# NVlabs/geomapnet

Hardware: AMD Instinct MI355X
Metric: images/sec MapNet ResNet-34 256x341 T=3 train step (higher is better)
Workload: dtype f16 (MFMA operands f16, f32 accumulate; forward conv operands as f16 pairs hi + lo, 3 MFMAs per product; backward 1 MFMA per product)

## Files before the change

### geomapnet_amd/_binding.py

```python
import ctypes as C
import os

_HERE = os.path.dirname(os.path.abspath(__file__))
LIB_PATH = os.path.join(_HERE, "libmapnet_hip.so")

c_void = C.c_void_p
c_f = C.c_float
c_i = C.c_int
c_i64 = C.c_int64


class Entry(C.Structure):
    _fields_ = [("name", C.c_char * 96), ("offset", c_i64), ("numel", c_i64), ("ndim", C.c_int32),
                ("shape", C.c_int32 * 4), ("is_buffer", C.c_int32), ("is_int64", C.c_int32), ("ohwi", C.c_int32),
                ("stage", C.c_int32)]


class Config(C.Structure):
    _fields_ = [("mode", C.c_int32), ("dtype", C.c_int32), ("windows", C.c_int32), ("T", C.c_int32), ("H", C.c_int32),
                ("W", C.c_int32), ("feat_dim", C.c_int32), ("filter_nans", C.c_int32), ("loss_scale", c_f),
                ("eps_mode", C.c_int32)]


class GatherGeom(C.Structure):
# ... 3 lines not shown

_PROTOS = {
    "mn_last_error": (C.c_char_p, []),
    "mn_backend": (C.c_char_p, []),
    "mn_model_entries": (c_i, [c_i]),
    "mn_model_entry": (c_i, [c_i, c_i, C.POINTER(Entry)]),
    "mn_model_param_floats": (c_i64, [c_i]),
    "mn_model_buffer_bytes": (c_i64, [c_i]),
    "mn_plan_bytes": (c_i64, [C.POINTER(Config)]),
    "mn_create": (c_void, [C.POINTER(Config), c_void, c_void, c_void, c_void, c_void]),
    "mn_destroy": (None, [c_void]),
    "mn_set_learn_flags": (c_i, [c_void, c_i, c_i]),
    "mn_set_loss_fn": (c_i, [c_void, c_i, c_f, c_i, c_f]),
    "mn_set_optim": (c_i, [c_void, c_f, c_f, c_f, c_f, c_f, c_f]),
    "mn_set_optim_method": (c_i, [c_void, c_i, c_i]),
    "mn_set_step_count": (c_i, [c_void, c_i64]),
    "mn_get_step_count": (c_i64, [c_void]),
    "mn_stuck_overflow_steps": (c_i64, [c_void]),
    "mn_set_loss_host": (c_i, [c_void, c_void]),
    "mn_wait_loss": (c_i, [c_void]),
    "mn_set_loss_scale": (c_i, [c_void, c_f, c_i]),
    "mn_get_loss_scale": (c_i, [c_void, C.POINTER(c_f), C.POINTER(c_i64)]),
    "mn_debug_tensor": (c_i, [c_void, C.c_char_p, C.POINTER(c_void), C.POINTER(c_i64), C.POINTER(C.c_int32)]),
    "mn_set_dropout": (c_i, [c_void, c_f, C.c_uint64]),
    "mn_set_dropout_calls": (c_i, [c_void, C.c_uint32]),
    "mn_set_input_u8": (c_i, [c_void, c_i, C.POINTER(c_f), C.POINTER(c_f)]),
    "mn_set_color_jitter": (c_i, [c_void, c_f, c_f, c_f, c_f, C.c_uint64]),
    "mn_set_color_jitter_calls": (c_i, [c_void, C.c_uint32]),
    "mn_input_resize_bytes": (c_i64, [C.POINTER(Config), c_i, c_i]),
    "mn_set_input_resize": (c_i, [c_void, c_i, c_i, c_void, c_i64]),
    "mn_forward": (c_i, [c_void, c_void, c_void, c_i, c_void]),
    "mn_input_grad": (c_i, [c_void, c_void, c_void, c_void, c_void, c_void, c_void]),
    "mn_loss": (c_i, [c_void, c_void, c_void, c_void, c_void]),
    "mn_train_step": (c_i, [c_void, c_void, c_void, c_void, c_void, c_void]),
    "mn_train_forward_loss": (c_i, [c_void, c_void, c_void, c_void, c_void, c_void]),
    "mn_train_backward_stage": (c_i, [c_void, c_i, c_void]),
    "mn_grad_bucket": (c_i, [c_void, c_i, C.POINTER(c_i64), C.POINTER(c_i64)]),
    "mn_optim_step": (c_i, [c_void, c_f, c_void]),
    "mn_grad_bucket_pack_bf16": (c_i, [c_void, c_i, c_void, c_void]),
    "mn_grad_bucket_unpack_bf16": (c_i, [c_void, c_i, c_void, c_void]),
    "mn_params_changed": (c_i, [c_void]),
    "mn_set_profiling": (c_i, [c_void, c_i]),
    "mn_last_kernel_ms": (c_i, [c_void, c_i, C.POINTER(c_f), C.POINTER(c_i)]),
    "mn_op_igemm": (c_i, [c_i, C.POINTER(GatherGeom), c_void, c_void, c_void, c_i, c_void, c_void, c_i, c_void, c_void,
                          c_f, c_void, c_void]),
    "mn_op_igemm_grid_m": (c_i, [c_i]),
    "mn_op_wgrad": (c_i, [c_i, C.POINTER(GatherGeom), c_void, c_i, c_void, c_void, c_i, c_void, c_f, c_i, c_void, c_void]),
    "mn_op_wgrad_ws_floats": (c_i64, []),
    "mn_op_wgrad_ws": (c_i, [c_i, C.POINTER(GatherGeom), c_void, c_i, c_void, c_void, c_i, c_f, c_void, c_i64, c_void, c_void]),
    "mn_op_conv_halo_pp": (c_i, [C.POINTER(GatherGeom), c_void, c_void, c_void, c_i, c_void, c_i, c_i, c_void, c_void, c_void, c_f,
                                 c_i, c_void]),
    "mn_op_conv_halo_pp_h2gates": (c_i, [C.POINTER(GatherGeom), c_void, c_void, c_void, c_i, c_void, c_i, c_i, c_void, c_void, c_void,
                                         c_f, c_i, c_void]),
    "mn_op_conv_halo_h2": (c_i, [C.POINTER(GatherGeom), c_void, c_void, c_void, c_i, c_void, c_i, c_void]),
    "mn_op_conv_dgrad": (c_i, [c_i, c_i, c_i, c_i, c_i, c_i, c_i, c_i, c_i, c_void, c_void, c_void, c_void, c_void, c_void, c_i,
                               c_void, c_void]),
    "mn_op_stem_conv": (c_i, [c_void, c_void, c_void, c_void, c_i, c_i, c_i, c_i, c_i, c_void]),
    "mn_op_stem_conv_x3": (c_i, [c_void, c_void, c_void, c_void, c_i, c_i, c_i, c_i, c_i, c_void]),
    "mn_op_dense": (c_i, [c_void, c_void, c_void, c_void, c_i, c_i, c_i, c_i, c_void]),
    "mn_op_dense_wgrad": (c_i, [c_void, c_void, c_void, c_void, c_i, c_i, c_i, c_f, c_void]),
    "mn_op_head_wgrad": (c_i, [c_void, c_void, c_void, c_void, c_void, c_void, c_i, c_i, c_f, c_i, c_void]),
    "mn_op_stem_bwd": (c_i, [c_void, c_void, c_void, c_void, c_void, c_void, c_void, c_void, c_void, c_i, c_void, c_void, c_void,
                             c_void, c_void, c_i, c_i, c_i, c_i, c_f, c_void]),
    "mn_op_stem_bwd_pregated": (c_i, [c_void, c_void, c_void, c_void, c_void, c_void, c_void, c_void, c_void, c_i, c_void, c_void,
                                      c_void, c_void, c_void, c_i, c_i, c_i, c_i, c_f, c_void]),
    "mn_op_oihw_to_ohwi": (c_i, [c_void, c_void, c_i, c_i, c_i, c_i, c_i, c_void]),
    "mn_op_criterion": (c_i, [c_i, c_i, c_i, c_void, c_void, c_void, c_void, c_void, c_void, c_void, c_f, c_void]),
    "mn_op_criterion_fn": (c_i, [c_i, c_i, c_i, c_void, c_void, c_void, c_void, c_void, c_void, c_void, c_f, c_i, c_f, c_i, c_f,
                                 c_void]),
    "mn_op_calc_vos": (c_i, [c_void, c_i, c_i, c_void, c_void, c_void, c_void]),
    "mn_pgo_optimize": (c_i, [c_void, c_void, c_void, c_void, c_i, c_i, c_i, C.c_double, C.c_double, C.c_double,
                              C.c_double, c_i, c_void]),
    "mn_op_adam": (c_i, [c_void, c_void, c_void, c_void, c_i64, c_i64, c_f, c_f, c_f, c_f, c_f, c_i64, c_f, c_f, c_void,
                         c_i, c_void]),
    "mn_op_optim": (c_i, [c_i, c_i, c_void, c_void, c_void, c_void, c_i64, c_i64, c_f, c_f, c_f, c_f, c_f, c_i64, c_f, c_f, c_void,
                          c_i, c_void]),
    "mn_op_bn_train_fwd": (c_i, [c_i, c_void, c_i64, c_i, c_void, c_void, c_void, c_void, c_void, c_void, c_void, c_i,
                                 c_void, c_f, c_f, c_void, c_void]),
    "mn_op_bn_bwd": (c_i, [c_i, c_void, c_void, c_void, c_i64, c_i, c_void, c_void, c_void, c_void, c_void, c_void, c_void,
                           c_void, c_f, c_void]),
    "mn_op_bn_train_fwd_h2": (c_i, [c_void, c_i64, c_i, c_void, c_void, c_void, c_void, c_void, c_void, c_void, c_i, c_void, c_void,
                                    c_f, c_f, c_void, c_void]),
    "mn_op_bn_bwd_rows": (c_i, [c_i, c_void, c_void, c_void, c_i64, c_i, c_void, c_void, c_void, c_void, c_void, c_void, c_void,
                                c_void, c_void, c_i, c_f, c_void]),
    "mn_op_bn_relu_maxpool_h2": (c_i, [c_void, c_void, c_void, c_void, c_void, c_i, c_i, c_i, c_i, c_void]),
    "mn_op_avgpool_fwd_h2": (c_i, [c_void, c_void, c_i, c_i, c_i, c_void]),
    "mn_op_avgpool_bwd": (c_i, [c_i, c_void, c_void, c_void, c_i, c_i, c_i, c_void]),
    "mn_op_widen_f16": (c_i, [c_void, c_void, c_i64, c_void]),
    "mn_op_maxpool_fwd": (c_i, [c_i, c_void, c_void, c_void, c_i, c_i, c_i, c_i, c_void]),
    "mn_op_maxpool_bwd": (c_i, [c_i, c_void, c_void, c_void, c_i, c_i, c_i, c_i, c_void]),
    "mn_op_occupy": (c_i, [c_i, c_i, c_f, c_void, c_void, c_i64, c_i, c_void]),
    "mn_op_color_jitter": (c_i, [c_void, c_void, c_void, c_void, c_i, c_i, c_i, C.POINTER(c_f), C.c_uint64, C.c_uint32,
                                 C.POINTER(c_f), C.POINTER(c_f), c_void]),
    "mn_op_resize_u8": (c_i, [c_void, c_void, c_void, c_i, c_i, c_i, c_i, c_i, c_void]),
    "mn_op_resize_work_bytes": (c_i64, [c_i, c_i, c_i, c_i]),
    "mn_op_resize_tile": (c_i, [c_i, c_i, c_i, c_i, C.POINTER(c_i), C.POINTER(c_i)]),
    "mn_op_stem_dgrad": (c_i, [c_i, c_void, c_void, c_void, c_i, c_i, c_i, c_f, c_void]),
    "mn_op_bn_eval_bwd": (c_i, [c_i, c_void, c_void, c_void, c_void, c_i64, c_i, c_void]),
    "mn_op_saliency": (c_i, [c_void, c_void, c_void, c_void, c_i, c_i, c_i, c_void]),
    "mn_op_saliency_work_floats": (c_i64, [c_i]),
}

SYMBOLS = tuple(_PROTOS)


class MapNetHipError(RuntimeError):
# ... 53 lines not shown
```

### geomapnet_amd/csrc/knobs.h

```cpp
#pragma once
#include <stdlib.h>

namespace mn {

constexpr int kKnobUnset = -0x7fffffff;

struct Knobs {
  bool deterministic = false;
  int fuse_stem = 1;
  bool wgrad_stream = true;
  bool early_fork = true;
  int wgrad_sched = kKnobUnset;
  int wgrad_early_stages = kKnobUnset;
  int wgrad_defer_stages = kKnobUnset;
  int wgrad_tail = 1;
  int scale_growth = 2000;

  int igemm_config = 0;
  int igemm_halo = 2;
  int halo384 = 1;
  int halo_a1 = 1;
  bool h2_halo256 = false;
  bool wgrad_fused = true;
  int stem_wgs = 0;
  int halo_pp_wgs = 256;
  int halo_h2_wgs = 256;

#ifdef MN_ABLATION_BUILD
  int ablate = 0;
  int wgf_ablate = 0;
  int halo_ablate = 0;
  int halo_pp_ablate = 0;
  int halo_h2_ablate = 0;
  int abl_skip_finalize = 0;
  bool abl_skip_wgf = false;
  bool wgf_skip_reduce = false;
#endif
};

namespace knob_env {
inline int integer(const char* name, int dflt) {
  const char* e = getenv(name);
  return e ? atoi(e) : dflt;
}
inline bool on_unless_0(const char* name) { return integer(name, 1) != 0; }
inline bool present(const char* name) { return getenv(name) != nullptr; }
}

inline Knobs& knobs_storage() {
  static Knobs k;
  return k;
}
inline const Knobs& knobs() { return knobs_storage(); }

inline void load_knobs() {
  using namespace knob_env;
  Knobs k;
  k.deterministic = integer("MN_DETERMINISTIC", 0) != 0;
  k.fuse_stem = integer("MN_FUSE_STEM", k.fuse_stem);
  k.wgrad_stream = on_unless_0("MN_WGRAD_STREAM");
  k.early_fork = on_unless_0("MN_EARLY_FORK");
  k.wgrad_sched = integer("MN_WGRAD_SCHED", kKnobUnset);
  k.wgrad_early_stages = integer("MN_WGRAD_EARLY_STAGES", kKnobUnset);
  k.wgrad_defer_stages = integer("MN_WGRAD_DEFER_STAGES", kKnobUnset);
  k.wgrad_tail = integer("MN_WGRAD_TAIL", k.wgrad_tail);
  k.scale_growth = integer("MN_SCALE_GROWTH", k.scale_growth);
  k.igemm_config = integer("MN_IGEMM_CONFIG", k.igemm_config);
  k.igemm_halo = integer("MN_IGEMM_HALO", k.igemm_halo);
  k.halo384 = integer("MN_HALO384", k.halo384);
  k.halo_a1 = integer("MN_HALO_A1", k.halo_a1);
  k.h2_halo256 = integer("MN_H2_HALO256", 0) != 0;
  k.wgrad_fused = on_unless_0("MN_WGRAD_FUSED");
  k.stem_wgs = integer("MN_STEM_WGS", k.stem_wgs);
  k.halo_pp_wgs = integer("MN_HALO_PP_WGS", k.halo_pp_wgs);
  k.halo_h2_wgs = integer("MN_HALO_H2_WGS", k.halo_h2_wgs);
#ifdef MN_ABLATION_BUILD
  k.ablate = integer("MN_ABLATE", 0);
  k.wgf_ablate = integer("MN_WGF_ABLATE", 0);
  k.halo_ablate = integer("MN_HALO_ABLATE", 0);
  k.halo_pp_ablate = integer("MN_HALO_PP_ABLATE", 0);
  k.halo_h2_ablate = integer("MN_HALO_H2_ABLATE", 0);
  k.abl_skip_finalize = integer("MN_ABL_SKIP_FINALIZE", 0);
  k.abl_skip_wgf = present("MN_ABL_SKIP_WGF");
  k.wgf_skip_reduce = present("MN_WGF_SKIP_REDUCE");
#endif
  knobs_storage() = k;
}

struct WgradSchedule {
  int sched, early_stages, defer_stages;
};
inline WgradSchedule resolve_wgrad_schedule(const Knobs& k, bool f16_family, bool per_stage) {
  WgradSchedule r;
  r.sched = k.wgrad_sched != kKnobUnset ? k.wgrad_sched : !k.early_fork ? 0 : f16_family ? 1 : 2;
  r.early_stages = k.wgrad_early_stages != kKnobUnset ? k.wgrad_early_stages : per_stage ? 13 : 15;
  r.defer_stages = k.wgrad_defer_stages != kKnobUnset ? k.wgrad_defer_stages : per_stage ? 2 : 0;
  return r;
}

}
```

### geomapnet_amd/csrc/net.hip

```cpp
#include "../../include/mapnet_hip.h"

#include <cmath>
#include <cstring>
#include <deque>
#include <memory>
#include <string>
#include <vector>

#include "common.h"
#include "criterion.h"
#include "elementwise.h"
#include "elementwise_h2.h"
#include "head.h"
#include "jitter.h"
#include "resize.h"
#include "knobs.h"
#include "dense.h"
#include "igemm.h"
#include "dgrad.h"
#include "halo_pp.h"
#include "input_grad.h"
#include "layout.h"
#include "optim.h"
#include "pool.h"
#include "stem.h"
#include "stem_bwd.h"
#include "util.h"
#include "wgrad.h"

using namespace mn;

static const Layout& layout_for(int feat_dim) {
  static thread_local std::unique_ptr<Layout> cache;
  if (!cache || cache->feat_dim != feat_dim) cache.reset(new Layout(feat_dim));
  return *cache;
}
extern "C" int mn_model_entries(int feat_dim) { return (int)layout_for(feat_dim).entries.size(); }
extern "C" int mn_model_entry(int feat_dim, int idx, mn_entry* out) {
  const Layout& L = layout_for(feat_dim);
  if (idx < 0 || idx >= (int)L.entries.size()) return fail("mn_model_entry: index out of range");
  *out = L.entries[idx];
  return 0;
}
extern "C" int64_t mn_model_param_floats(int feat_dim) { return layout_for(feat_dim).param_floats; }
extern "C" int64_t mn_model_buffer_bytes(int feat_dim) { return layout_for(feat_dim).buffer_bytes; }

namespace {

struct Bump {
  size_t cur = 0;
  size_t take(size_t bytes) {
    size_t o = cur;
    cur += (bytes + 255) & ~(size_t)255;
    return o;
  }
};

struct KernelTimer {
  bool enabled = false;
  struct Pair {
    hipEvent_t a, b;
    int cat;
  };
  std::deque<Pair> pool;
  size_t used = 0;
  float ms[4] = {0, 0, 0, 0};
  int launches[4] = {0, 0, 0, 0};
  Pair* begin(int cat, hipStream_t s) {
    if (!enabled) return nullptr;
    if (used == pool.size()) {
      Pair p;
      hipEventCreate(&p.a);
      hipEventCreate(&p.b);
// ... 554 lines not shown
  }
  void launch_repack(int first_block, int n_blocks, int n_jobs, hipStream_t s) {
    void (*kernel)(const RepackJob*, int, const float*, int) = repack_all_kernel<T>;
    if constexpr (DT == MN_F32) {
      if (md.wf == FMT_H2Q)
        kernel = repack_all_kernel<float, true, true, true>;
      else if (md.wf == FMT_H2 && md.wd == FMT_F16)
        kernel = repack_all_kernel<float, true, true>;
      else if (md.wf == FMT_H2)
        kernel = repack_all_kernel<float, true>;
    }
    hipLaunchKernelGGL(kernel, dim3(n_blocks), dim3(256), 0, s, (const RepackJob*)repack_jobs, n_jobs, (const float*)params,
                       first_block);
  }

  BnParams bn_params(const Unit& u) {
    BnParams p;
    p.gamma = params + u.bp.gamma;
    p.beta = params + u.bp.beta;
    p.running_mean = (float*)buffers + u.bp.rm;
    p.running_var = (float*)buffers + u.bp.rv;
    p.num_batches_tracked = (long long*)(buffers + u.bp.nbt);
    p.mean = u.mean;
    p.invstd = u.invstd;
    p.eps = 1e-5f;
    p.momentum = 0.1f;
    return p;
  }
  static Epilogue plain_epilogue(void* out, int ldc) {
    Epilogue ep;
    ep.out = out; ep.ldc = ldc; ep.stats = nullptr; ep.bias = nullptr; ep.relu = 0; ep.res = nullptr; ep.res_gate = nullptr;
    ep.alpha = 1.f;
    return ep;
  }
  static GatherGeom dense_geom(int M, int N, int K) {
    GatherGeom g;
    g.B = M; g.Hi = 1; g.Wi = 1; g.C = K; g.P = 1; g.Q = 1; g.R = 1; g.S = 1; g.mul_p = 1; g.mul_q = 1; g.rsign = 1;
    g.ssign = 1; g.off_h = 0; g.off_w = 0; g.div = 1; g.M = M; g.N = N; g.K = K;
    return g;
  }
  Epilogue stats_epilogue(Unit& u, int training) {
    Epilogue ep = plain_epilogue(u.y, u.cp.cout);
    if (training) {
      ep.stats_accum = u.accum_f;
      ep.stats_rows = u.rows_f;
    }
    return ep;
  }
  void conv_bn_stats(Unit& u, const T* x, int training, hipStream_t s) {
    const Epilogue ep = stats_epilogue(u, training);
    auto* tp = timer.begin(0, s);
    if (md.pairs())
      launch_igemm_h2(u.gf, (const half*)x, (const half*)u.wf, ep, s, (const half*)zero_page, md.act == FMT_H2Q);
    else if (halo_path(u.gf) && conv_halo_pp_applies(u.gf, ep))
      launch_conv_halo_pp(u.gf, (const half*)x, (const half*)u.wf, ep, s);
    else
      launch_igemm<T>(u.gf, x, u.wf, ep, s, (const T*)zero_page);
    timer.end(tp, s);
  }
  void stem_conv(int training, hipStream_t s) {
    double* const sums = training ? stem.accum_f : nullptr;
    auto* tp = timer.begin(0, s);
    if (DT == MN_F32 && md.mma_fwd == MMA_F16X3)
      launch_stem_conv_x3((const float*)xpad, (const float*)stem.wf, (float*)stem.y, sums, stem.rows_f, B, H, W, Wp, s);
    else if (DT == MN_F16)
      launch_stem_conv((const half*)xpad, (const half*)stem.wf, (half*)stem.y, sums, stem.rows_f, B, H, W, Wp, s);
    else
      launch_igemm<T>(stem.gf, xpad, stem.wf, stats_epilogue(stem, training), s, (const T*)zero_page);
    timer.end(tp, s);
  }
  bool halo_path(const GatherGeom& g) const { return md.act == FMT_F16 && conv_halo_applies(g); }
  void bn_finalize(Unit& u, hipStream_t s) {
#ifdef MN_ABLATION_BUILD
    const int skip_c = knobs().abl_skip_finalize;
    static long calls = 0;
    if (u.cp.cout <= skip_c && ++calls > 400) return;
#endif
    hipLaunchKernelGGL(bn_finalize_fwd_kernel, dim3(cdiv(u.cp.cout, kBnFinalizeChannels)), dim3(256), 0, s, (const double*)u.accum_f, (double)u.M,
                       bn_params(u), cur_training, u.coef_f, u.cp.cout, u.rows_f);
  }
  void bn_act(Unit& u, const T* res, int relu, T* out, hipStream_t s) {
    long np = u.M * u.cp.cout / VEC;
    bn_finalize(u, s);
    if (md.pairs()) {
      const long ni = u.M * u.cp.cout / 8;
      hipLaunchKernelGGL(bn_apply_h2_kernel, dim3(ew_grid(ni)), dim3(256), 0, s, (const float*)u.y, (const float*)u.coef_f,
                         (const half*)res, (half*)out, ni, u.cp.cout, relu, md.act == FMT_H2Q ? 1 : 0,
                         cur_training ? u.rec : (half*)nullptr, (const float*)u.mean, (const float*)u.invstd);
      return;
    }
    hipLaunchKernelGGL((bn_apply_kernel<T>), dim3(ew_grid(np)), dim3(256), 0, s, (const T*)u.y, (const float*)u.coef_f, res, out,
                       np, u.cp.cout, relu);
  }

  void launch_jitter_input(const unsigned char* images, half* x16, hipStream_t s) {
    launch_u8_jitter<T>(images, xpad, B, H, W, Hp, Wp, jitter_norm, x16, jitter_params(jit_range, jit_seed, jit_calls), jit_draws,
                        jit_partials, jit_mean, s);
    jit_calls += 1;
  }

  int forward(const void* images, float* poses_out, int training, hipStream_t s) override {
    return forward_impl(images, poses_out, training, false, s);
  }
  int forward_impl(const void* images, float* poses_out, int training, bool zero_grads, hipStream_t s) {
    if (jitter_on() && !input_u8)
      return fail("forward: ColorJitter (mn_set_color_jitter) needs uint8 input (mn_set_input_u8): fp32 frames arrive already "
                  "normalised, and ColorJitter must come before Normalize");
    if (resize_on && !input_u8)
// ... 109 lines not shown
    if (int e = forward_impl(images, poses_out, 1, true, s)) return e;
    cur_targets = targets;
    cur_loss = loss_out ? loss_out : loss_dev;
    return 0;
  }

  void bn_bwd(Unit& u, const T* g, hipStream_t s, bool self_gate = false) {
    float* const gamma = params + u.bp.gamma;
    const float* const sg_beta = self_gate ? params + u.bp.beta : nullptr;
    if (md.f16_bwd_on_pairs())
      launch_bn_bwd_rec((const half*)g, (const half*)u.rec, u.M, u.cp.cout, gamma, u.mean, u.invstd, grads + u.bp.gamma,
                        grads + u.bp.beta, (half*)u.gy, u.accum_b, u.coef_b, 1.f / cur_scale, s, self_gate, u.rows_b);
    else if (md.gy == FMT_H2)
      launch_bn_bwd_h2((const float*)g, (const float*)u.y, u.M, u.cp.cout, gamma, u.mean, u.invstd, grads + u.bp.gamma,
                       grads + u.bp.beta, (half*)u.gy, u.accum_b, u.coef_b, 1.f / cur_scale, s, sg_beta, u.rows_b);
    else
      launch_bn_bwd<T>(g, (const T*)nullptr, (const T*)u.y, u.M, u.cp.cout, gamma, u.mean, u.invstd, grads + u.bp.gamma,
                       grads + u.bp.beta, u.gy, u.accum_b, u.coef_b, 1.f / cur_scale, s, sg_beta, PoolGradSrc(), u.rows_b);
  }
  WgradArgs wgrad_args(Unit& u, const T* x) {
    WgradArgs a;
    a.g = u.gf; a.dY = u.gy; a.ldy = u.cp.cout; a.X = x; a.dW = grads + u.cp.w; a.ldw = u.ldw; a.colmap = u.colmap;
    a.g.mma = md.mma_bwd;
    a.alpha = 1.f / cur_scale; a.rows_per_split = 0;
    a.ws = wgf_ws; a.ws_floats = wgf_ws_floats;
    a.det = deterministic;
    return a;
  }
  static int wgrad_splits(const Unit& u) { return u.cp.cout >= 128 ? 512 : (u.M > 2000000 ? 2048 : 1024); }
  void conv_wgrad(Unit& u, const T* x, hipStream_t ws) {
    WgradArgs a = wgrad_args(u, x);
    auto* tp = timer.begin(1, ws);
    if (md.f16_bwd_on_pairs()) {
      a.g.mma = MMA_NATIVE;
      a.x_h2 = true;
      launch_wgrad<half>(a, wgrad_splits(u), ws, zero_page);
    } else if (md.gy == FMT_H2) {
      a.g.mma = MMA_H2;
      launch_wgrad<half>(a, wgrad_splits(u), ws, zero_page);
    } else {
      launch_wgrad<T>(a, wgrad_splits(u), ws, zero_page);
    }
    timer.end(tp, ws);
  }
  void conv_dgrad(Unit& u, T* gx, const T* res, hipStream_t s, const T* out_gate = nullptr) {
    Epilogue ep = plain_epilogue(gx, u.cp.cin);
    ep.res = res;
    ep.out_gate = out_gate;
    auto* tp = timer.begin(0, s);
    if (md.gy == FMT_H2) {
      launch_conv_dgrad<half>(u.dg, (const half*)u.gy, (const half*)u.wd, ep, s, (const half*)zero_page, parity_dgrad, true);
    } else if (md.gy == FMT_F16) {
      ep.gate_h2 = md.pairs();
      if (conv_halo_applies(u.dg.full) && conv_halo_pp_applies(u.dg.full, ep))
        launch_conv_halo_pp(u.dg.full, (const half*)u.gy, (const half*)u.wd, ep, s);
      else
        launch_conv_dgrad<half>(u.dg, (const half*)u.gy, (const half*)u.wd, ep, s, (const half*)zero_page, parity_dgrad);
    } else {
      launch_conv_dgrad<T>(u.dg, (const T*)u.gy, (const T*)u.wd, ep, s, (const T*)zero_page, parity_dgrad);
    }
    timer.end(tp, s);
  }
  void block_input_dgrad(Block& blk, const T* below, hipStream_t s) {
    if (blk.down) {
      conv_dgrad(blk.u1, blk.gx, nullptr, s, below);
      conv_dgrad(blk.ud, blk.gx, blk.gx, s, below);
    } else {
      conv_dgrad(blk.u1, blk.gx, blk.gout, s, below);
    }
  }
  void flush_wgrads(hipStream_t s) {
    if (pending_wgrads.empty()) return;
    hipStream_t ws = fork_wgrad(s);
    for (auto& p : pending_wgrads) conv_wgrad(*p.u, p.x, ws);
    pending_wgrads.clear();
  }
  void block_backward(Block& blk, hipStream_t s) {
    const T* bx = blk.x;
    const T* ba1 = blk.a1;
    const T* below = &blk == &blocks.front() ? (md.stem_bwd == STEM_TILES_ON_COPIES ? bx : nullptr) : bx;
    if (wgrad.sched == 2 || ((wgrad.defer_stages >> blk.stage) & 1)) {
      flush_wgrads(s);
      bn_bwd(blk.u2, blk.gout, s);
      conv_dgrad(blk.u2, blk.ga1, nullptr, s);
      pending_wgrads.push_back({&blk.u2, ba1});
      flush_wgrads(s);
      bn_bwd(blk.u1, blk.ga1, s, true);
      if (blk.down) bn_bwd(blk.ud, blk.gout, s);
      pending_wgrads.push_back({&blk.u1, bx});
      if (blk.down) pending_wgrads.push_back({&blk.ud, bx});
      block_input_dgrad(blk, below, s);
      return;
    }
    bn_bwd(blk.u2, blk.gout, s);
    const bool tail = blk.stage == 0 && !blk.down && (int)(&blk - &blocks[0]) < wgrad_tail;
    const bool early = wgrad.sched == 1 && !tail && ((wgrad.early_stages >> blk.stage) & 1);
    if (early) conv_wgrad(blk.u2, ba1, fork_wgrad(s));
    conv_dgrad(blk.u2, blk.ga1, nullptr, s);
    bn_bwd(blk.u1, blk.ga1, s, true);
    if (blk.down) bn_bwd(blk.ud, blk.gout, s);
    if (tail) {
      pending_wgrads.push_back({&blk.u2, ba1});
      pending_wgrads.push_back({&blk.u1, bx});
    } else {
      hipStream_t ws = fork_wgrad(s);
      if (!early) conv_wgrad(blk.u2, ba1, ws);
      conv_wgrad(blk.u1, bx, ws);
      if (blk.down) conv_wgrad(blk.ud, bx, ws);
// ... 584 lines not shown
```

### geomapnet_amd/csrc/ops.hip

```cpp
#include "../../include/mapnet_hip.h"

#include <string>

#include "common.h"
#include "criterion.h"
#include "elementwise.h"
#include "elementwise_h2.h"
#include "head.h"
#include "jitter.h"
#include "knobs.h"
#include "dense.h"
#include "igemm.h"
#include "dgrad.h"
#include "halo_pp.h"
#include "input_grad.h"
#include "optim.h"
#include "pgo.h"
#include "pool.h"
#include "rehearsal.h"
#include "resize.h"
#include "stem.h"
#include "stem_bwd.h"
#include "wgrad.h"
#include "util.h"

using namespace mn;

namespace mn {
thread_local std::string g_last_error;
}

extern "C" const char* mn_last_error(void) { return mn::g_last_error.c_str(); }

#ifndef MN_BACKEND_NAME
#define MN_BACKEND_NAME "hip"
#endif
extern "C" const char* mn_backend(void) { return MN_BACKEND_NAME; }

static void begin_op() {
  begin_call();
  load_knobs();
}

static GatherGeom to_geom(const mn_gather_geom* g) {
  GatherGeom r;
  r.B = g->B; r.Hi = g->Hi; r.Wi = g->Wi; r.C = g->C; r.P = g->P; r.Q = g->Q; r.R = g->R; r.S = g->S;
  r.mul_p = g->mul_p; r.mul_q = g->mul_q; r.rsign = g->rsign; r.ssign = g->ssign;
  r.off_h = g->off_h; r.off_w = g->off_w; r.div = g->div; r.M = g->M; r.N = g->N; r.K = g->K;
  return r;
}

static int check_geom(const GatherGeom& g, int dtype) {
  int vec = dtype == MN_F16 ? 8 : 4;
  if ((dtype == MN_DTYPE_F16X2 || dtype == MN_DTYPE_F16X2Q) && (g.C % 32 != 0 || g.N % 4 != 0))
    return fail("igemm: h2 operands need C % 32 == 0");
  if (g.C % vec != 0) return fail("igemm: C must be a multiple of the 16-byte piece");
  if (g.K != g.R * g.S * g.C) return fail("igemm: K != R*S*C");
  if (g.K % (4 * vec) != 0) return fail("igemm: K must be a multiple of the 64-byte K-step");
  if (g.M != g.B * g.P * g.Q) return fail("igemm: M != B*P*Q");
  if (g.div != 1 && g.div != 2) return fail("igemm: div must be 1 or 2");
  if (g.div == 2 && (g.rsign != -1 || g.ssign != -1)) return fail("igemm: div = 2 requires rsign = ssign = -1");
  if (g.R * g.S > 32) return fail("igemm: at most 32 taps");
  if ((long)g.B * g.Hi * g.Wi * g.C >= (1L << 31)) return fail("igemm: A tensor exceeds 2^31 elements");
  return 0;
}

extern "C" int mn_op_igemm_grid_m(int M) { return igemm_grid_m(M); }

extern "C" int mn_op_igemm(int dtype, const mn_gather_geom* gg, const void* A, const void* Bw, void* out, int ldc,
                           float* stats, const float* bias, int relu, const void* res, const void* res_gate, float alpha,
                           const void* zero_page, void* stream) {
  begin_op();
  GatherGeom g = to_geom(gg);
  if (int e = check_geom(g, dtype)) return e;
  if (!zero_page) return fail("igemm: zero_page (>= 16 zero bytes of device memory) is required");
  {
    const long es = dtype == MN_DTYPE_F16 ? 2 : 4;
    if ((long)gg->B * gg->Hi * gg->Wi * gg->C * es >= 0xfffffff0l || (long)gg->N * gg->K * es >= 0xfffffff0l)
      return fail("igemm: operands must be smaller than 4 GiB (32-bit buffer offsets)");
  }
  Epilogue ep;
  ep.out = out; ep.ldc = ldc; ep.stats = stats; ep.bias = bias; ep.relu = relu; ep.res = res; ep.res_gate = res_gate;
  ep.alpha = alpha;
  if (dtype == MN_DTYPE_F32X3) g.mma = MMA_F16X3;
  if (dtype == MN_DTYPE_F16X2 || dtype == MN_DTYPE_F16X2Q) {
    launch_igemm_h2(g, (const half*)A, (const half*)Bw, ep, (hipStream_t)stream, (const half*)zero_page, dtype == MN_DTYPE_F16X2Q);
    return check_launch("igemm");
  }
  if (dtype == MN_F16)
    launch_igemm<half>(g, (const half*)A, (const half*)Bw, ep, (hipStream_t)stream, (const half*)zero_page);
  else
    launch_igemm<float>(g, (const float*)A, (const float*)Bw, ep, (hipStream_t)stream, (const float*)zero_page);
  return check_launch("igemm");
}

static int op_conv_halo_pp(const mn_gather_geom* gg, const void* A, const void* Bw, void* out, int ldc, double* stats_accum,
                           int stats_rows, int relu, const void* res, const void* res_gate, const void* out_gate, float alpha, int wgs,
                           bool gate_h2, void* stream) {
  begin_op();
  GatherGeom g = to_geom(gg);
  if (int e = check_geom(g, MN_F16)) return e;
  Epilogue ep;
  ep.out = out; ep.ldc = ldc; ep.stats = nullptr; ep.bias = nullptr; ep.relu = relu; ep.res = res; ep.res_gate = res_gate;
  ep.out_gate = out_gate; ep.alpha = alpha; ep.stats_accum = stats_accum; ep.stats_rows = stats_rows;
  ep.gate_h2 = gate_h2;
  if (!conv_halo_pp_applies(g, ep))
    return fail("conv_halo_pp: fp16 3x3 stride-1 same-size convolutions of 64 -> 64 channels only (stats_rows > 0 with stats_accum)");
  launch_conv_halo_pp(g, (const half*)A, (const half*)Bw, ep, (hipStream_t)stream, wgs);
  return check_launch("conv_halo_pp");
}
extern "C" int mn_op_conv_halo_pp(const mn_gather_geom* gg, const void* A, const void* Bw, void* out, int ldc, double* stats_accum,
                                 int stats_rows, int relu, const void* res, const void* res_gate, const void* out_gate,
                                 float alpha, int wgs, void* stream) {
  return op_conv_halo_pp(gg, A, Bw, out, ldc, stats_accum, stats_rows, relu, res, res_gate, out_gate, alpha, wgs, false, stream);
}
extern "C" int mn_op_conv_halo_pp_h2gates(const mn_gather_geom* gg, const void* A, const void* Bw, void* out, int ldc,
                                          double* stats_accum, int stats_rows, int relu, const void* res, const void* res_gate,
                                          const void* out_gate, float alpha, int wgs, void* stream) {
  return op_conv_halo_pp(gg, A, Bw, out, ldc, stats_accum, stats_rows, relu, res, res_gate, out_gate, alpha, wgs, true, stream);
}

static int op_wgrad(int dtype, const mn_gather_geom* gg, const void* dY, int ldy, const void* X, float* dW, int ldw,
                    const int32_t* colmap, float alpha, int target_blocks, const void* zero_page, float* ws, long ws_floats,
                    void* stream);
extern "C" int mn_op_conv_halo_h2(const mn_gather_geom* gg, const void* A, const void* Bw, float* out, int ldc, double* stats_accum,
                                  int stats_rows, void* stream) {
  begin_op();
  GatherGeom g = to_geom(gg);
  if (int e = check_geom(g, MN_DTYPE_F16X2)) return e;
  Epilogue ep;
  ep.out = out; ep.ldc = ldc; ep.stats = nullptr; ep.bias = nullptr; ep.relu = 0; ep.res = nullptr; ep.res_gate = nullptr;
  ep.out_gate = nullptr; ep.alpha = 1.f; ep.stats_accum = stats_accum; ep.stats_rows = stats_rows;
  if (!conv_halo_h2_applies(g, ep))
    return fail("conv_halo_h2: 3x3 stride-1 same-size forward convolutions of 64 -> 64 channel h2 tensors only (stats_rows > 0 with stats_accum)");
  launch_conv_halo_h2(g, (const half*)A, (const half*)Bw, ep, (hipStream_t)stream);
  return check_launch("conv_halo_h2");
}

extern "C" int mn_op_wgrad(int dtype, const mn_gather_geom* gg, const void* dY, int ldy, const void* X, float* dW, int ldw,
                           const int32_t* colmap, float alpha, int target_blocks, const void* zero_page, void* stream) {
  return op_wgrad(dtype, gg, dY, ldy, X, dW, ldw, colmap, alpha, target_blocks, zero_page, nullptr, 0, stream);
}
extern "C" int64_t mn_op_wgrad_ws_floats(void) { return wgrad_fused_ws_floats(WGF_BLOCKS); }
extern "C" int mn_op_wgrad_ws(int dtype, const mn_gather_geom* gg, const void* dY, int ldy, const void* X, float* dW, int ldw,
                              float alpha, float* ws, int64_t ws_floats, const void* zero_page, void* stream) {
  if (!ws || ws_floats <= 0) return fail("wgrad_ws: workspace required (mn_op_wgrad_ws_floats() floats)");
  return op_wgrad(dtype, gg, dY, ldy, X, dW, ldw, nullptr, alpha, 512, zero_page, ws, (long)ws_floats, stream);
}
static int op_wgrad(int dtype, const mn_gather_geom* gg, const void* dY, int ldy, const void* X, float* dW, int ldw,
                    const int32_t* colmap, float alpha, int target_blocks, const void* zero_page, float* ws, long ws_floats,
                    void* stream) {
  begin_op();
  WgradArgs a;
  a.ws = ws;
  a.ws_floats = ws_floats;
  a.g = to_geom(gg);
  if (dtype < MN_DTYPE_F32 || dtype > MN_DTYPE_F16X2M)
    return fail("wgrad: dtype must be MN_DTYPE_F32, _F16, _F32X3, _F16X2 or _F16X2M");
  const bool mixed = dtype == MN_DTYPE_F16X2M;
  int vec = dtype == MN_F16 || mixed ? 8 : 4;
  if (a.g.C % vec != 0 || a.g.N % vec != 0) return fail("wgrad: channel counts must be multiples of the piece");
  if (dtype == MN_DTYPE_F16X2 && (a.g.C % 32 != 0 || ldy % 32 != 0)) return fail("wgrad: h2 operands need channel counts % 32 == 0");
  if (mixed && a.g.C % 32 != 0) return fail("wgrad: an h2 X operand needs C % 32 == 0");
  a.dY = dY; a.ldy = ldy; a.X = X; a.dW = dW; a.ldw = ldw; a.colmap = colmap; a.alpha = alpha; a.rows_per_split = 0;
  if (dtype == MN_DTYPE_F32X3) a.g.mma = MMA_BF16X3;
  if (dtype == MN_DTYPE_F16X2) a.g.mma = MMA_H2;
  a.x_h2 = mixed;
  if (dtype == MN_F16 || dtype == MN_DTYPE_F16X2 || mixed)
    launch_wgrad<half>(a, target_blocks, (hipStream_t)stream, zero_page);
  else
    launch_wgrad<float>(a, target_blocks, (hipStream_t)stream);
  return check_launch("wgrad");
// ... 522 lines not shown
```

### include/mapnet_hip.h

```cpp
#ifndef MAPNET_HIP_H
#define MAPNET_HIP_H
#include <stddef.h>
#include <stdint.h>

#ifdef __cplusplus
extern "C" {
#endif

enum { MN_DTYPE_F32 = 0, MN_DTYPE_F16 = 1, MN_DTYPE_F32X3 = 2, MN_DTYPE_F16X2 = 3, MN_DTYPE_F16X2M = 4, MN_DTYPE_F16X2Q = 5 };
enum {
  MN_MODE_POSENET = 0,
  MN_MODE_MAPNET = 1,
  MN_MODE_MAPNET_ONLINE = 2,
  MN_MODE_MAPNET_GPS = 3
};
enum mn_loss_kind {
  MN_LOSS_L1 = 0,
  MN_LOSS_MSE = 1,
  MN_LOSS_SMOOTH_L1 = 2,
  MN_LOSS_HUBER = 3,
  MN_LOSS_QUATERNION = 4
};

const char* mn_last_error(void);
// ... 56 lines not shown

int mn_set_color_jitter(mn_handle* h, float brightness, float contrast, float saturation, float hue, uint64_t seed);
int mn_set_color_jitter_calls(mn_handle* h, uint32_t calls);

int64_t mn_input_resize_bytes(const mn_config* cfg, int src_h, int src_w);
int mn_set_input_resize(mn_handle* h, int src_h, int src_w, void* work, int64_t work_bytes);

int mn_input_grad(mn_handle* h, const void* images, const float* cot, float* gx_out, float* saliency_out, float* poses_out,
                  void* stream);

int mn_loss(mn_handle* h, const float* pred, const float* targ, float* loss_out, void* stream);

int mn_train_step(mn_handle* h, const void* images, const float* targets, float* loss_out, float* poses_out,
                  void* stream);

int mn_train_forward_loss(mn_handle* h, const void* images, const float* targets, float* loss_out,
                          float* poses_out, void* stream);
int mn_train_backward_stage(mn_handle* h, int stage, void* stream);
int mn_grad_bucket(mn_handle* h, int stage, int64_t* offset, int64_t* count);
int mn_optim_step(mn_handle* h, float grad_mul, void* stream);
int mn_grad_bucket_pack_bf16(mn_handle* h, int stage, void* out_bf16, void* stream);
int mn_grad_bucket_unpack_bf16(mn_handle* h, int stage, const void* in_bf16, void* stream);

int mn_set_loss_scale(mn_handle* h, float scale, int growth_interval);
int mn_get_loss_scale(mn_handle* h, float* scale, int64_t* skipped_steps);
int64_t mn_stuck_overflow_steps(mn_handle* h);

int mn_debug_tensor(mn_handle* h, const char* name, void** ptr, int64_t* numel, int32_t* dtype);

int mn_params_changed(mn_handle* h);

int mn_set_profiling(mn_handle* h, int enable);
int mn_last_kernel_ms(mn_handle* h, int which, float* ms, int* launches);

typedef struct mn_gather_geom {
  int32_t B, Hi, Wi, C, P, Q, R, S, mul_p, mul_q, rsign, ssign, off_h, off_w, div, M, N, K;
} mn_gather_geom;

int mn_op_igemm(int dtype, const mn_gather_geom* g, const void* A, const void* Bw, void* out, int ldc, float* stats,
                const float* bias, int relu, const void* res, const void* res_gate, float alpha, const void* zero_page,
                void* stream);
int mn_op_igemm_grid_m(int M);
int mn_op_wgrad(int dtype, const mn_gather_geom* g, const void* dY, int ldy, const void* X, float* dW, int ldw,
                const int32_t* colmap, float alpha, int target_blocks, const void* zero_page, void* stream);
int64_t mn_op_wgrad_ws_floats(void);
int mn_op_wgrad_ws(int dtype, const mn_gather_geom* g, const void* dY, int ldy, const void* X, float* dW, int ldw, float alpha,
                   float* ws, int64_t ws_floats, const void* zero_page, void* stream);
int mn_op_conv_halo_pp(const mn_gather_geom* g, const void* A, const void* Bw, void* out, int ldc, double* stats_accum,
                       int stats_rows, int relu, const void* res, const void* res_gate, const void* out_gate, float alpha,
                       int wgs, void* stream);
int mn_op_conv_halo_pp_h2gates(const mn_gather_geom* g, const void* A, const void* Bw, void* out, int ldc, double* stats_accum,
                               int stats_rows, int relu, const void* res, const void* res_gate, const void* out_gate, float alpha,
                               int wgs, void* stream);
int mn_op_conv_halo_h2(const mn_gather_geom* g, const void* A, const void* Bw, float* out, int ldc, double* stats_accum,
                       int stats_rows, void* stream);
int mn_op_conv_dgrad(int dtype, int B, int Hin, int Win, int Cin, int Cout, int k, int stride, int pad, const void* gy,
                     const void* wd, void* gx, const void* res, const void* res_gate, const void* out_gate, int parity,
                     const void* zero_page, void* stream);
int mn_op_stem_conv(const void* xpad, const void* wf, void* y, double* stats_accum, int stats_rows, int B, int H, int W, int Wp,
                    void* stream);
int mn_op_stem_conv_x3(const float* xpad, const float* wf, float* y, double* stats_accum, int stats_rows, int B, int H, int W,
                       int Wp, void* stream);
int mn_op_dense(const float* A, const float* W, const float* bias, float* C, int M, int N, int K, int relu, void* stream);
int mn_op_dense_wgrad(const float* dY, const float* X, float* dW, float* db, int B, int F, int Cin, float alpha, void* stream);
int mn_op_head_wgrad(const float* dposes, const float* feat, float* dWx, float* dbx, float* dWq, float* dbq, int B, int K, float scale,
                     int filter_nans, void* stream);
int mn_op_stem_bwd(const void* y, const unsigned char* idx, const void* gp, const float* gamma, const float* beta,
                   const float* mean, const float* invstd, const void* xpad, float* dW, int ldw, const int32_t* colmap,
                   float* dgamma, float* dbeta, float* coef_scratch, double* accum_scratch, int B, int H, int W, int Wp,
                   float alpha, void* stream);
int mn_op_stem_bwd_pregated(const void* y, const unsigned char* idx, const void* gp, const float* gamma, const float* beta,
                            const float* mean, const float* invstd, const void* xpad, float* dW, int ldw, const int32_t* colmap,
                            float* dgamma, float* dbeta, float* coef_scratch, double* accum_scratch, int B, int H, int W, int Wp,
                            float alpha, void* stream);
int mn_op_oihw_to_ohwi(const float* src, float* dst, int O, int I, int H, int W, int to_ohwi, void* stream);

int mn_op_criterion(int mode, int N, int T, const float* pred, const float* targ, const float* s, float* loss,
                    float* dpred, float* ds, float* vos_out, float grad_scale, void* stream);
int mn_op_criterion_fn(int mode, int N, int T, const float* pred, const float* targ, const float* s, float* loss,
                       float* dpred, float* ds, float* vos_out, float grad_scale, int t_kind, float t_param, int q_kind,
                       float q_param, void* stream);
int mn_op_calc_vos(const float* poses, int N, int T, float* vos, const float* cot, float* dposes, void* stream);

int mn_pgo_optimize(const double* poses, const double* vos, double* out, int32_t* status, int W, int N, int fc_vos,
                    double sax, double saq, double srx, double srq, int n_iters, void* stream);

int mn_op_adam(float* p, const float* g, float* m, float* v, int64_t n, int64_t n_clip, float lr, float wd,
               float beta1, float beta2, float eps, int64_t step, float grad_mul, float max_norm, double* sqnorm_scratch,
               int eps_mode, void* stream);
int mn_op_optim(int method, int nesterov, float* p, const float* g, float* m, float* v, int64_t n, int64_t n_clip, float lr,
                float wd, float beta1, float beta2, float eps, int64_t step, float grad_mul, float max_norm,
                double* sqnorm_scratch, int eps_mode, void* stream);

int mn_op_bn_train_fwd(int dtype, const void* y, int64_t M, int C, const float* gamma, const float* beta,
                       float* running_mean, float* running_var, float* mean, float* invstd, const void* res,
                       int relu, void* out, float eps, float momentum, double* accum_scratch, void* stream);
int mn_op_bn_bwd(int dtype, const void* g, const void* gate, const void* y, int64_t M, int C, const float* gamma,
                 const float* mean, const float* invstd, float* dgamma, float* dbeta, void* gy, float* coef_scratch,
                 double* accum_scratch, float grad_unscale, void* stream);
int mn_op_bn_bwd_rows(int dtype, const void* g, const void* gate, const void* y, int64_t M, int C, const float* gamma,
                      const float* beta, const float* mean, const float* invstd, float* dgamma, float* dbeta, void* gy,
                      float* coef_scratch, double* accum_scratch, int accum_rows, float grad_unscale, void* stream);
int mn_op_bn_train_fwd_h2(const float* y, int64_t M, int C, const float* gamma, const float* beta, float* running_mean,
                          float* running_var, float* mean, float* invstd, const void* res, int relu, void* out, void* rec, float eps,
                          float momentum, double* accum_scratch, void* stream);
int mn_op_bn_relu_maxpool_h2(const float* y, const float* coef, void* out, unsigned char* idx, void* y16, int B, int H, int W, int C,
// ... 28 lines not shown
```

Baseline: 10570.

## Add register-resident-weight halo conv kernel for 64-channel 3x3 dgrad

Adds a new persistent 3x3 64->64 fp16 convolution kernel. Each thread keeps all 72 weight fragments in registers, tiles the output as 8x16, and double-buffers the halo input tile in shared memory, with the next tile's loads interleaved among the MFMAs. By default it replaces the previous halo_pp kernel only on the backward dgrad path (knob bit 1). The forward use sits behind bit 2, which is off by default. The aim is to cut repeated weight traffic from LDS/global and hide the halo loads, at the cost of very high register pressure and one workgroup per CU.

```diff
diff --git a/geomapnet_amd/_binding.py b/geomapnet_amd/_binding.py
--- a/geomapnet_amd/_binding.py
+++ b/geomapnet_amd/_binding.py
@@ -79,6 +79,10 @@
                                  c_i, c_void]),
     "mn_op_conv_halo_pp_h2gates": (c_i, [C.POINTER(GatherGeom), c_void, c_void, c_void, c_i, c_void, c_i, c_i, c_void, c_void, c_void,
                                          c_f, c_i, c_void]),
+    "mn_op_conv_halo_r": (c_i, [C.POINTER(GatherGeom), c_void, c_void, c_void, c_i, c_void, c_i, c_i, c_void, c_void, c_void, c_f,
+                                c_i, c_void]),
+    "mn_op_conv_halo_r_h2gates": (c_i, [C.POINTER(GatherGeom), c_void, c_void, c_void, c_i, c_void, c_i, c_i, c_void, c_void, c_void,
+                                        c_f, c_i, c_void]),
     "mn_op_conv_halo_h2": (c_i, [C.POINTER(GatherGeom), c_void, c_void, c_void, c_i, c_void, c_i, c_void]),
     "mn_op_conv_dgrad": (c_i, [c_i, c_i, c_i, c_i, c_i, c_i, c_i, c_i, c_i, c_void, c_void, c_void, c_void, c_void, c_void, c_i,
                                c_void, c_void]),
diff --git a/geomapnet_amd/csrc/halo_r.h b/geomapnet_amd/csrc/halo_r.h
--- /dev/null
+++ b/geomapnet_amd/csrc/halo_r.h
@@ -0,0 +1,248 @@
+#pragma once
+#include "halo_pp.h"
+
+namespace mn {
+
+constexpr int kRTH = 8, kRTW = 16;
+constexpr int kRHW = kRTW + 2, kRHPIX = (kRTH + 2) * kRHW;
+constexpr int kRPieces = kRHPIX * 8;
+constexpr int kRPasses = (kRPieces + 255) / 256;
+constexpr int kRBuf = (kRPieces + 63) / 64 * 64;
+
+template <bool STATS, bool SIDE, int PD = 3>
+static __global__ void __launch_bounds__(256, 1) conv_halo_r_kernel(GatherGeom g, const half* __restrict__ A,
+                                                                    const half* __restrict__ Bw, Epilogue ep, int tiles_x,
+                                                                    int tiles_y, int ntiles) {
+  static_assert(!(STATS && SIDE), "the statistics form takes no residual / gates (conv_halo_pp_applies)");
+  constexpr int TH = kRTH, TW = kRTW, HW = kRHW;
+  constexpr unsigned kOob = 0x80000000u;
+  __shared__ piece_t smem[2 * kRBuf];
+
+  const int t = threadIdx.x, lane = t & 63;
+  const int wave = __builtin_amdgcn_readfirstlane(t >> 6);
+  const int l31 = lane & 31, kh = lane >> 5;
+  const int G = gridDim.x;
+  const int wl = xcd_remap(blockIdx.x, G);
+  const int nitems = wl < ntiles ? (ntiles - wl + G - 1) / G : 0;
+  const bool flip = g.rsign < 0;
+  const int gP = g.P, gQ = g.Q, gHi = g.Hi, gWi = g.Wi;
+  const int off_h = flip ? g.off_h - 2 : g.off_h, off_w = flip ? g.off_w - 2 : g.off_w;
+  const float alpha = ep.alpha;
+  const bool relu = (ep.relu & 1) != 0;
+
+  const long tensor_bytes = (long)g.B * g.P * g.Q * 64L * 2L;
+  const __amdgpu_buffer_rsrc_t rsrc_a = make_rsrc(A, (long)g.B * g.Hi * g.Wi * 64L * 2L);
+  const __amdgpu_buffer_rsrc_t rsrc_out = make_rsrc(ep.out, tensor_bytes);
+  const __amdgpu_buffer_rsrc_t rsrc_res = make_rsrc(ep.res, ep.res ? tensor_bytes : 0L);
+  const int gmul = ep.gate_h2 ? 2 : 1;
+  const void* const gate_ptr = ep.res_gate ? ep.res_gate : ep.out_gate;
+  const __amdgpu_buffer_rsrc_t rsrc_g1 = make_rsrc(gate_ptr, gate_ptr ? tensor_bytes * gmul : 0L);
+  const bool has_res = SIDE && ep.res != nullptr, has_gate = SIDE && ep.res_gate != nullptr;
+  const bool has_ogate = SIDE && ep.out_gate != nullptr;
+
+  PieceView<half> wr[72];
+  {
+    const half* row = Bw + (long)l31 * g.K + kh * 8;
+#pragma unroll
+    for (int i = 0; i < 72; ++i) {
+      const int pos = i >> 3, ks = (i >> 1) & 3, jj = i & 1;
+      const int tap = flip ? 8 - pos : pos;
+      wr[i].p = *reinterpret_cast<const piece_t*>(row + (long)jj * 32 * g.K + tap * 64 + ks * 16);
+    }
+  }
+
+  auto tile_coords = [&](int tile, int& b, int& y0, int& x0) __attribute__((always_inline)) {
+    const int txi = tile % tiles_x;
+    const int tmp = tile / tiles_x;
+    const int tyi = tmp % tiles_y;
+    b = tmp / tiles_y;
+    y0 = tyi * TH;
+    x0 = txi * TW;
+  };
+  int nb = 0, ny0 = 0, nx0 = 0;
+  auto halo_pass = [&](int i, int buf) __attribute__((always_inline)) {
+    if (i * 256 + wave * 64 >= kRPieces) return;
+    const int oy = ny0 + off_h, ox = nx0 + off_w;
+    const int sidx = i * 256 + t;
+    const int hp = sidx >> 3, slot = sidx & 7;
+    const int hy = hp / HW, hx = hp - hy * HW;
+    const int iy = oy + hy, ix = ox + hx;
+    const bool ok = hp < kRHPIX && (unsigned)iy < (unsigned)gHi && (unsigned)ix < (unsigned)gWi;
+    const unsigned off = ok ? (unsigned)(((nb * gHi + iy) * gWi + ix) * 128 + ((slot ^ ((hx >> 1) & 7)) << 4)) : ~0u;
+    dma16(rsrc_a, off, 0u, &smem[buf * kRBuf + i * 256 + wave * 64]);
+  };
+
+  floatx16 acc[2];
+  float st1[STATS ? 2 : 1][16], st2[STATS ? 2 : 1][16];
+  if constexpr (STATS) {
+#pragma unroll
+    for (int jj = 0; jj < 2; ++jj)
+#pragma unroll
+      for (int r = 0; r < 16; ++r) st1[jj][r] = st2[jj][r] = 0.f;
+  }
+
+  const int col = l31 & 15, prow = 2 * wave + (l31 >> 4);
+  const unsigned lane_pix = (unsigned)((prow * gQ + col) * 128);
+  int cb = 0, cy0 = 0, cx0 = 0;
+  auto pixel_ok = [&]() __attribute__((always_inline)) { return cy0 + prow < gP && cx0 + col < gQ; };
+  auto tile_base = [&]() __attribute__((always_inline)) { return ((cb * gP + cy0) * gQ + cx0) * 128; };
+  Half4View rv[SIDE ? 2 : 1][4], gv[SIDE ? 2 : 1][4];
+  auto side_load = [&](int k) __attribute__((always_inline)) {
+    if constexpr (SIDE) {
+      const int jj = (k >> 2) & 1, q = k & 3;
+      const bool ok = pixel_ok();
+      if (k < 8)
+        rv[jj][q].p = __builtin_amdgcn_raw_buffer_load_b64(rsrc_res, (int)(ok ? lane_pix + kh * 8 : kOob), tile_base() + jj * 64 + q * 16, 0);
+      else
+        gv[jj][q].p = __builtin_amdgcn_raw_buffer_load_b64(rsrc_g1, (int)(ok ? lane_pix * gmul + kh * 8 : kOob),
+                                                           (tile_base() + jj * 64) * gmul + q * 16, 0);
+    }
+  };
+
+  const unsigned pbase = (unsigned)((prow * HW + col) * 128);
+  unsigned xs[3];
+#pragma unroll
+  for (int dx = 0; dx < 3; ++dx) xs[dx] = (unsigned)((kh ^ (((col + dx) >> 1) & 7)) << 4);
+
+  auto compute = [&](int buf, bool next) __attribute__((always_inline)) {
+    const char* hb = reinterpret_cast<const char*>(&smem[buf * kRBuf]);
+#pragma unroll
+    for (int jj = 0; jj < 2; ++jj)
+#pragma unroll
+      for (int r = 0; r < 16; ++r) acc[jj][r] = 0.f;
+    constexpr int NS = 36;
+    PieceView<half> fb[PD + 1];
+    auto load_frag = [&](int j) __attribute__((always_inline)) {
+      const int dy = j % 3, grp = j / 3;
+      const int ks = grp & 3, dx = grp >> 2;
+      const char* pp = hb + (pbase + (unsigned)(dx * 128) + ((unsigned)(ks * 32) ^ xs[dx]));
+      fb[j % (PD + 1)].p = *reinterpret_cast<const piece_t*>(pp + dy * HW * 128);
+    };
+#pragma unroll
+    for (int j = 0; j < PD; ++j) load_frag(j);
+#pragma unroll
+    for (int j = 0; j < NS; ++j) {
+      const int dy = j % 3, grp = j / 3;
+      const int i = ((dy * 3 + (grp >> 2)) * 4 + (grp & 3)) * 2;
+      const int sl = j % (PD + 1);
+      mma_piece<half>(wr[i], fb[sl], acc[0]);
+      __builtin_amdgcn_sched_barrier(0);
+      if (j + PD < NS) load_frag(j + PD);
+      __builtin_amdgcn_sched_barrier(0);
+      mma_piece<half>(wr[i + 1], fb[sl], acc[1]);
+      __builtin_amdgcn_sched_barrier(0);
+      constexpr int D0 = SIDE ? 16 : 0;
+      if (SIDE && j < 16) side_load(j);
+      if (next && j >= D0 && j < D0 + kRPasses) halo_pass(j - D0, buf ^ 1);
+      __builtin_amdgcn_sched_barrier(0);
+    }
+  };
+
+  auto store = [&]() __attribute__((always_inline)) {
+    const bool okp = pixel_ok();
+    const unsigned voff = okp ? lane_pix + kh * 8 : kOob;
+    const int sbase = tile_base();
+#pragma unroll
+    for (int jj = 0; jj < 2; ++jj)
+#pragma unroll
+      for (int q = 0; q < 4; ++q) {
+        Half4View o;
+#pragma unroll
+        for (int e = 0; e < 4; ++e) {
+          const int r = q * 4 + e;
+          float v = acc[jj][r] * alpha;
+          if (relu) v = fmaxf(v, 0.f);
+          if constexpr (STATS) {
+            const float vs = okp ? v : 0.f;
+            st1[jj][r] += vs;
+            st2[jj][r] += vs * vs;
+          }
+          if constexpr (SIDE) {
+            if (has_res) {
+              float xr = (float)rv[jj][q].e[e];
+              if (has_gate && !((float)gv[jj][q].e[e] > 0.f)) xr = 0.f;
+              v += xr;
+            }
+            if (has_ogate && !((float)gv[jj][q].e[e] > 0.f)) v = 0.f;
+          }
+          o.e[e] = (half)v;
+        }
+        __builtin_amdgcn_raw_buffer_store_b64(o.p, rsrc_out, (int)voff, sbase + jj * 64 + q * 16, 0);
+      }
+  };
+
+  if (nitems > 0) {
+    tile_coords(wl, nb, ny0, nx0);
+#pragma unroll
+    for (int i = 0; i < kRPasses; ++i) halo_pass(i, 0);
+  }
+  wait_vmcnt<0>();
+  __builtin_amdgcn_s_barrier();
+  for (int p = 0; p < nitems; ++p) {
+    const int buf = p & 1;
+    const bool next = p + 1 < nitems;
+    tile_coords(wl + p * G, cb, cy0, cx0);
+    if (next) tile_coords(wl + (p + 1) * G, nb, ny0, nx0);
+    compute(buf, next);
+    wait_vmcnt<0>();
+    store();
+    __builtin_amdgcn_s_barrier();
+  }
+  wait_vmcnt<0>();
+
+  if constexpr (STATS) {
+    if (ep.stats_accum && nitems > 0) {
+      float* red = reinterpret_cast<float*>(&smem[0]);
+#pragma unroll
+      for (int jj = 0; jj < 2; ++jj)
+#pragma unroll
+        for (int r = 0; r < 16; ++r) {
+          float a = st1[jj][r], bsum = st2[jj][r];
+#pragma unroll
+          for (int o = 16; o > 0; o >>= 1) {
+            a += __shfl_xor(a, o);
+            bsum += __shfl_xor(bsum, o);
+          }
+          if (l31 == 0) {
+            const int n = jj * 32 + (r & 3) + 8 * (r >> 2) + 4 * kh;
+            red[(wave * 64 + n) * 2 + 0] = a;
+            red[(wave * 64 + n) * 2 + 1] = bsum;
+          }
+        }
+      __syncthreads();
+      if (t < 64) {
+        float sa = 0.f, sb = 0.f;
+#pragma unroll
+        for (int w = 0; w < 4; ++w) {
+          sa += red[(w * 64 + t) * 2 + 0];
+          sb += red[(w * 64 + t) * 2 + 1];
+        }
+        double* row = ep.stats_accum + (long)((int)blockIdx.x % ep.stats_rows) * 2 * 64;
+        atomicAdd(row + t, (double)sa);
+        atomicAdd(row + 64 + t, (double)sb);
+      }
+    }
+  }
+}
+
+inline bool conv_halo_r_applies(const GatherGeom& g, const Epilogue& ep) { return conv_halo_pp_applies(g, ep); }
+
+inline int conv_halo_r_grid(const GatherGeom& g, int wgs_arg = 0) {
+  const int ntiles = g.B * cdiv(g.P, kRTH) * cdiv(g.Q, kRTW);
+  const int wgs = wgs_arg > 0 ? wgs_arg : device_cus();
+  return ntiles < wgs ? ntiles : wgs;
+}
+inline void launch_conv_halo_r(const GatherGeom& g, const half* A, const half* Bw, const Epilogue& ep, hipStream_t stream,
+                               int wgs_arg = 0) {
+  const int tx = cdiv(g.Q, kRTW), ty = cdiv(g.P, kRTH);
+  const int ntiles = g.B * tx * ty;
+  const dim3 grid(conv_halo_r_grid(g, wgs_arg));
+  if (ep.stats_accum)
+    hipLaunchKernelGGL((conv_halo_r_kernel<true, false>), grid, dim3(256), 0, stream, g, A, Bw, ep, tx, ty, ntiles);
+  else if (ep.res || ep.res_gate || ep.out_gate)
+    hipLaunchKernelGGL((conv_halo_r_kernel<false, true>), grid, dim3(256), 0, stream, g, A, Bw, ep, tx, ty, ntiles);
+  else
+    hipLaunchKernelGGL((conv_halo_r_kernel<false, false>), grid, dim3(256), 0, stream, g, A, Bw, ep, tx, ty, ntiles);
+}
+
+}
diff --git a/geomapnet_amd/csrc/knobs.h b/geomapnet_amd/csrc/knobs.h
--- a/geomapnet_amd/csrc/knobs.h
+++ b/geomapnet_amd/csrc/knobs.h
@@ -25,6 +25,7 @@
   int stem_wgs = 0;
   int halo_pp_wgs = 256;
   int halo_h2_wgs = 256;
+  int halo_r = 1;
 
 #ifdef MN_ABLATION_BUILD
   int ablate = 0;
@@ -74,6 +75,7 @@
   k.stem_wgs = integer("MN_STEM_WGS", k.stem_wgs);
   k.halo_pp_wgs = integer("MN_HALO_PP_WGS", k.halo_pp_wgs);
   k.halo_h2_wgs = integer("MN_HALO_H2_WGS", k.halo_h2_wgs);
+  k.halo_r = integer("MN_HALO_R", k.halo_r);
 #ifdef MN_ABLATION_BUILD
   k.ablate = integer("MN_ABLATE", 0);
   k.wgf_ablate = integer("MN_WGF_ABLATE", 0);
diff --git a/geomapnet_amd/csrc/net.hip b/geomapnet_amd/csrc/net.hip
--- a/geomapnet_amd/csrc/net.hip
+++ b/geomapnet_amd/csrc/net.hip
@@ -19,6 +19,7 @@
 #include "igemm.h"
 #include "dgrad.h"
 #include "halo_pp.h"
+#include "halo_r.h"
 #include "input_grad.h"
 #include "layout.h"
 #include "optim.h"
@@ -679,8 +680,12 @@
     auto* tp = timer.begin(0, s);
     if (md.pairs())
       launch_igemm_h2(u.gf, (const half*)x, (const half*)u.wf, ep, s, (const half*)zero_page, md.act == FMT_H2Q);
-    else if (halo_path(u.gf) && conv_halo_pp_applies(u.gf, ep))
-      launch_conv_halo_pp(u.gf, (const half*)x, (const half*)u.wf, ep, s);
+    else if (halo_path(u.gf) && conv_halo_pp_applies(u.gf, ep)) {
+      if ((knobs().halo_r & 2) != 0 && !(deterministic && ep.stats_accum))
+        launch_conv_halo_r(u.gf, (const half*)x, (const half*)u.wf, ep, s);
+      else
+        launch_conv_halo_pp(u.gf, (const half*)x, (const half*)u.wf, ep, s);
+    }
     else
       launch_igemm<T>(u.gf, x, u.wf, ep, s, (const T*)zero_page);
     timer.end(tp, s);
@@ -896,8 +901,12 @@
       launch_conv_dgrad<half>(u.dg, (const half*)u.gy, (const half*)u.wd, ep, s, (const half*)zero_page, parity_dgrad, true);
     } else if (md.gy == FMT_F16) {
       ep.gate_h2 = md.pairs();
-      if (conv_halo_applies(u.dg.full) && conv_halo_pp_applies(u.dg.full, ep))
-        launch_conv_halo_pp(u.dg.full, (const half*)u.gy, (const half*)u.wd, ep, s);
+      if (conv_halo_applies(u.dg.full) && conv_halo_pp_applies(u.dg.full, ep)) {
+        if ((knobs().halo_r & 1) != 0)
+          launch_conv_halo_r(u.dg.full, (const half*)u.gy, (const half*)u.wd, ep, s);
+        else
+          launch_conv_halo_pp(u.dg.full, (const half*)u.gy, (const half*)u.wd, ep, s);
+      }
       else
         launch_conv_dgrad<half>(u.dg, (const half*)u.gy, (const half*)u.wd, ep, s, (const half*)zero_page, parity_dgrad);
     } else {
diff --git a/geomapnet_amd/csrc/ops.hip b/geomapnet_amd/csrc/ops.hip
--- a/geomapnet_amd/csrc/ops.hip
+++ b/geomapnet_amd/csrc/ops.hip
@@ -13,6 +13,7 @@
 #include "igemm.h"
 #include "dgrad.h"
 #include "halo_pp.h"
+#include "halo_r.h"
 #include "input_grad.h"
 #include "optim.h"
 #include "pgo.h"
@@ -118,6 +119,32 @@
                                           double* stats_accum, int stats_rows, int relu, const void* res, const void* res_gate,
                                           const void* out_gate, float alpha, int wgs, void* stream) {
   return op_conv_halo_pp(gg, A, Bw, out, ldc, stats_accum, stats_rows, relu, res, res_gate, out_gate, alpha, wgs, true, stream);
+}
+
+static int op_conv_halo_r(const mn_gather_geom* gg, const void* A, const void* Bw, void* out, int ldc, double* stats_accum,
+                          int stats_rows, int relu, const void* res, const void* res_gate, const void* out_gate, float alpha, int wgs,
+                          bool gate_h2, void* stream) {
+  begin_op();
+  GatherGeom g = to_geom(gg);
+  if (int e = check_geom(g, MN_F16)) return e;
+  Epilogue ep;
+  ep.out = out; ep.ldc = ldc; ep.stats = nullptr; ep.bias = nullptr; ep.relu = relu; ep.res = res; ep.res_gate = res_gate;
+  ep.out_gate = out_gate; ep.alpha = alpha; ep.stats_accum = stats_accum; ep.stats_rows = stats_rows;
+  ep.gate_h2 = gate_h2;
+  if (!conv_halo_r_applies(g, ep))
+    return fail("conv_halo_r: fp16 3x3 stride-1 same-size convolutions of 64 -> 64 channels only (stats_rows > 0 with stats_accum)");
+  launch_conv_halo_r(g, (const half*)A, (const half*)Bw, ep, (hipStream_t)stream, wgs);
+  return check_launch("conv_halo_r");
+}
+extern "C" int mn_op_conv_halo_r(const mn_gather_geom* gg, const void* A, const void* Bw, void* out, int ldc, double* stats_accum,
+                                int stats_rows, int relu, const void* res, const void* res_gate, const void* out_gate,
+                                float alpha, int wgs, void* stream) {
+  return op_conv_halo_r(gg, A, Bw, out, ldc, stats_accum, stats_rows, relu, res, res_gate, out_gate, alpha, wgs, false, stream);
+}
+extern "C" int mn_op_conv_halo_r_h2gates(const mn_gather_geom* gg, const void* A, const void* Bw, void* out, int ldc,
+                                         double* stats_accum, int stats_rows, int relu, const void* res, const void* res_gate,
+                                         const void* out_gate, float alpha, int wgs, void* stream) {
+  return op_conv_halo_r(gg, A, Bw, out, ldc, stats_accum, stats_rows, relu, res, res_gate, out_gate, alpha, wgs, true, stream);
 }
 
 static int op_wgrad(int dtype, const mn_gather_geom* gg, const void* dY, int ldy, const void* X, float* dW, int ldw,
diff --git a/include/mapnet_hip.h b/include/mapnet_hip.h
--- a/include/mapnet_hip.h
+++ b/include/mapnet_hip.h
@@ -132,6 +132,12 @@
 int mn_op_conv_halo_pp_h2gates(const mn_gather_geom* g, const void* A, const void* Bw, void* out, int ldc, double* stats_accum,
                                int stats_rows, int relu, const void* res, const void* res_gate, const void* out_gate, float alpha,
                                int wgs, void* stream);
+int mn_op_conv_halo_r(const mn_gather_geom* g, const void* A, const void* Bw, void* out, int ldc, double* stats_accum,
+                      int stats_rows, int relu, const void* res, const void* res_gate, const void* out_gate, float alpha, int wgs,
+                      void* stream);
+int mn_op_conv_halo_r_h2gates(const mn_gather_geom* g, const void* A, const void* Bw, void* out, int ldc, double* stats_accum,
+                              int stats_rows, int relu, const void* res, const void* res_gate, const void* out_gate, float alpha,
+                              int wgs, void* stream);
 int mn_op_conv_halo_h2(const mn_gather_geom* g, const void* A, const void* Bw, float* out, int ldc, double* stats_accum,
                        int stats_rows, void* stream);
 int mn_op_conv_dgrad(int dtype, int B, int Hin, int Win, int Cin, int Cout, int k, int stride, int pad, const void* gy,
```

Result: no change. 10480 (-0.8%).
